# mikwieczorek/centroids-reid

Hardware: AMD Instinct MI355X
Metric: train_images_per_sec (higher is better)
Workload: dtype bf16; 1 GPU; ResNet50 256x128 CTL training step: fwd+bwd, centroid-triplet + center + xent, Adam + center SGD (BASELINE configs[1]); P=16, K=4, global_batch=64, num_classes=751, parallelism=single

## Files before the change

centroids-reid_amd/csrc/elementwise.hip:

```cpp
#include "conv_common.hpp"

#include "vec16.hpp"

template <int CW>
__global__ __launch_bounds__(1024) void bn2d_finalize_kernel(const float* __restrict__ partial, int rows, int C,
                                                            double count, float* __restrict__ rmean,
                                                            float* __restrict__ rvar, int training, float momentum,
                                                            float eps, const float* __restrict__ gamma,
                                                            const float* __restrict__ beta,
                                                            float* __restrict__ mean_out,
                                                            float* __restrict__ invstd_out,
                                                            float* __restrict__ scale_shift) {
  constexpr int RG = 1024 / CW;
  __shared__ double red[16][2][CW];
  const int cl = threadIdx.x % CW, rg = threadIdx.x / CW;
  const int c = blockIdx.x * CW + cl;
  if (!training) {
    if (rg == 0 && c < C) {
      const float mu = rmean[c], is = 1.0f / sqrtf(rvar[c] + eps);
      mean_out[c] = mu; invstd_out[c] = is;
      const float sc = is * (gamma ? gamma[c] : 1.f);
      scale_shift[c] = sc; scale_shift[C + c] = (beta ? beta[c] : 0.f) - mu * sc;
    }
    return;
// ... 472 lines not shown
    cb[k] = b.x; cb[k + 1] = b.y; cb[k + 2] = b.z; cb[k + 3] = b.w;
    cc[k] = c.x; cc[k + 1] = c.y; cc[k + 2] = c.z; cc[k + 3] = c.w;
  }
  if (!pg.dy && !act) {
    for (int64_t i = gtid; i < total; i += 2 * nthreads) {
      const int64_t i2 = i + nthreads;
      const bool two = i2 < total;
      float xv[V], gv[V], xw[V], gw[V];
      unsigned m1 = 0xffu, m2 = 0xffu;
      Vec16<T>::load(x + i * V, xv);
      Vec16<T>::load(g + i * V, gv);
      if (mask) m1 = mask[i];
      if (two) {
        Vec16<T>::load(x + i2 * V, xw);
        Vec16<T>::load(g + i2 * V, gw);
        if (mask) m2 = mask[i2];
      }
      float o[V];
#pragma unroll
      for (int k = 0; k < V; ++k) { gv[k] = ((m1 >> k) & 1u) ? gv[k] : 0.f; o[k] = fmaf(ca[k], gv[k], fmaf(cb[k], xv[k], cc[k])); }
      if (gm_out) Vec16<T>::store(gm_out + i * V, gv);
      Vec16<T>::store(dx + i * V, o);
      if (two) {
#pragma unroll
        for (int k = 0; k < V; ++k) { gw[k] = ((m2 >> k) & 1u) ? gw[k] : 0.f; o[k] = fmaf(ca[k], gw[k], fmaf(cb[k], xw[k], cc[k])); }
        if (gm_out) Vec16<T>::store(gm_out + i2 * V, gw);
        Vec16<T>::store(dx + i2 * V, o);
      }
    }
    return;
  }
  for (int64_t i = gtid; i < total; i += nthreads) {
    float xv[V], gv[V];
    Vec16<T>::load(x + i * V, xv);
    if (pg.dy) {
      const int64_t r = i / cpr;
      const int hw = pg.H * pg.W, bb = (int)(r / hw), rem = (int)(r - (int64_t)bb * hw);
      pool_grad_gather<T>(reinterpret_cast<const T*>(pg.dy), pg.idx, bb, rem / pg.W, rem % pg.W, (int)(i - r * cpr), pg.H / 2,
                          pg.W / 2, cpr, gv);
    } else {
      Vec16<T>::load(g + i * V, gv);
    }
    if (mask) {
      const unsigned m = mask[i];
#pragma unroll
      for (int k = 0; k < V; ++k) gv[k] = ((m >> k) & 1u) ? gv[k] : 0.f;
    } else if (act) {
      float av[V];
      Vec16<T>::load(act + i * V, av);
#pragma unroll
      for (int k = 0; k < V; ++k) gv[k] = av[k] > 0.f ? gv[k] : 0.f;
    }
    if (gm_out) Vec16<T>::store(gm_out + i * V, gv);
    float o[V];
#pragma unroll
    for (int k = 0; k < V; ++k) o[k] = fmaf(ca[k], gv[k], fmaf(cb[k], xv[k], cc[k]));
    Vec16<T>::store(dx + i * V, o);
  }
}

template <int V>
__device__ __forceinline__ void store_taps(uint8_t* p, const uint8_t (&bi)[V]) {
  static_assert(V == 4 || V == 8, "16-byte vectors of 4- or 2-byte elements");
  uint32_t lo = (uint32_t)bi[0] | ((uint32_t)bi[1] << 8) | ((uint32_t)bi[2] << 16) | ((uint32_t)bi[3] << 24);
  if constexpr (V == 4) {
    *reinterpret_cast<uint32_t*>(p) = lo;
  } else {
    uint32_t hi = (uint32_t)bi[4] | ((uint32_t)bi[5] << 8) | ((uint32_t)bi[6] << 16) | ((uint32_t)bi[7] << 24);
    *reinterpret_cast<uint2*>(p) = make_uint2(lo, hi);
  }
}
template <typename T>
__global__ __launch_bounds__(256) void maxpool_fwd_kernel(const T* __restrict__ x, int B, int H, int W, int C,
                                                          T* __restrict__ y, uint8_t* __restrict__ idx) {
  constexpr int V = Vec16<T>::N;
  const int OH = H / 2, OW = W / 2, cpr = C / V;
  const int64_t total = (int64_t)B * OH * OW * cpr;
  for (int64_t i = (int64_t)blockIdx.x * 256 + threadIdx.x; i < total; i += (int64_t)gridDim.x * 256) {
    int cc, ox, oy, b;
    if (total < (int64_t)1 << 31) {
      const unsigned u = (unsigned)i, q1 = u / (unsigned)cpr, q2 = q1 / (unsigned)OW;
      cc = (int)(u - q1 * cpr); ox = (int)(q1 - q2 * OW); b = (int)(q2 / (unsigned)OH); oy = (int)(q2 - (unsigned)b * OH);
    } else {
      cc = (int)(i % cpr);
      int64_t p = i / cpr;
      ox = (int)(p % OW); p /= OW;
      oy = (int)(p % OH);
      b = (int)(p / OH);
    }
    float best[V];
    uint8_t bi[V];
#pragma unroll
    for (int k = 0; k < V; ++k) { best[k] = -INFINITY; bi[k] = 0; }
#pragma unroll
    for (int r = 0; r < 3; ++r)
#pragma unroll
      for (int s = 0; s < 3; ++s) {
        const int iy = oy * 2 + r - 1, ix = ox * 2 + s - 1;
        if ((unsigned)iy < (unsigned)H && (unsigned)ix < (unsigned)W) {
          float v[V];
          Vec16<T>::load(x + (((int64_t)b * H + iy) * W + ix) * C + cc * V, v);
#pragma unroll
          for (int k = 0; k < V; ++k)
            if (v[k] > best[k]) { best[k] = v[k]; bi[k] = (uint8_t)(r * 3 + s); }
        }
      }
    Vec16<T>::store(y + i * V, best);
    if (idx) store_taps<V>(idx + i * V, bi);
  }
}

template <typename T>
__global__ __launch_bounds__(256) void bn_apply_maxpool_kernel(const T* __restrict__ x, const float* __restrict__ scale_shift,
                                                               int relu, int B, int H, int W, int C, T* __restrict__ y,
                                                               uint8_t* __restrict__ idx) {
  constexpr int V = Vec16<T>::N;
  const int OH = H / 2, OW = W / 2, cpr = C / V;
  const int64_t total = (int64_t)B * OH * OW * cpr;
  for (int64_t i = (int64_t)blockIdx.x * 256 + threadIdx.x; i < total; i += (int64_t)gridDim.x * 256) {
    int cc, ox, oy, b;
    if (total < (int64_t)1 << 31) {
      const unsigned u = (unsigned)i, q1 = u / (unsigned)cpr, q2 = q1 / (unsigned)OW;
      cc = (int)(u - q1 * cpr); ox = (int)(q1 - q2 * OW); b = (int)(q2 / (unsigned)OH); oy = (int)(q2 - (unsigned)b * OH);
    } else {
      cc = (int)(i % cpr);
      int64_t p = i / cpr;
      ox = (int)(p % OW); p /= OW;
      oy = (int)(p % OH);
      b = (int)(p / OH);
    }
    float sc[V], sh[V], best[V];
    uint8_t bi[V];
#pragma unroll
    for (int k = 0; k < V; ++k) { sc[k] = scale_shift[cc * V + k]; sh[k] = scale_shift[C + cc * V + k]; best[k] = -INFINITY; bi[k] = 0; }
#pragma unroll
    for (int r = 0; r < 3; ++r)
#pragma unroll
      for (int s = 0; s < 3; ++s) {
        const int iy = oy * 2 + r - 1, ix = ox * 2 + s - 1;
        if ((unsigned)iy < (unsigned)H && (unsigned)ix < (unsigned)W) {
          float v[V];
          Vec16<T>::load(x + (((int64_t)b * H + iy) * W + ix) * C + cc * V, v);
#pragma unroll
          for (int k = 0; k < V; ++k) {
            float yv = fmaf(v[k], sc[k], sh[k]);
            if (relu) yv = fmaxf(yv, 0.f);
            yv = Vec16<T>::rnd(yv);
            if (yv > best[k]) { best[k] = yv; bi[k] = (uint8_t)(r * 3 + s); }
          }
        }
      }
    Vec16<T>::store(y + i * V, best);
    if (idx) store_taps<V>(idx + i * V, bi);
  }
}

template <typename T>
__global__ __launch_bounds__(256) void maxpool_bwd_kernel(const T* __restrict__ dy, const uint8_t* __restrict__ idx,
                                                          int B, int H, int W, int C, T* __restrict__ dx) {
  constexpr int V = Vec16<T>::N;
  const int OH = H / 2, OW = W / 2, cpr = C / V;
  const int row = blockIdx.x;
  const int b = row / H, iy = row - b * H;
  T* drow = dx + (int64_t)row * W * C;
  const int nr = (iy & 1) ? 2 : 1;
  const int rr0 = (iy & 1) ? 0 : 1, rstep = 2;
  for (int par = 0; par < 2; ++par) {
    const int ns = par ? 2 : 1, ss0 = par ? 0 : 1;
    for (int v = threadIdx.x; v < (W / 2) * cpr; v += 256) {
      const int ix = 2 * (v / cpr) + par, cc = v % cpr;
      float acc[V];
#pragma unroll
      for (int k = 0; k < V; ++k) acc[k] = 0.f;
      for (int ri = 0; ri < nr; ++ri) {
        const int r = rr0 + ri * rstep, oy = (iy + 1 - r) >> 1;
        if (oy >= OH) continue;
        for (int si = 0; si < ns; ++si) {
          const int sx = ss0 + si * 2, ox = (ix + 1 - sx) >> 1;
          if (ox >= OW) continue;
          const int64_t o = ((((int64_t)b * OH + oy) * OW + ox) * cpr + cc) * V;
          float g[V];
          Vec16<T>::load(dy + o, g);
          uint8_t tap[V];
          if constexpr (V == 8) *reinterpret_cast<uint2*>(tap) = *reinterpret_cast<const uint2*>(idx + o);
          else *reinterpret_cast<unsigned*>(tap) = *reinterpret_cast<const unsigned*>(idx + o);
          const uint8_t want = (uint8_t)(r * 3 + sx);
#pragma unroll
          for (int k = 0; k < V; ++k) acc[k] += (tap[k] == want) ? g[k] : 0.f;
        }
      }
      Vec16<T>::store(drow + ((int64_t)ix * cpr + cc) * V, acc);
    }
  }
}

template <typename T>
__global__ __launch_bounds__(256) void gap_fwd_kernel(const T* __restrict__ x, int HW, int C, float* __restrict__ out,
                                                      int64_t* __restrict__ counter) {
  constexpr int V = Vec16<T>::N;
  __shared__ float red[8][32][V + 1];
  if (counter && blockIdx.x == 0 && blockIdx.y == 0 && threadIdx.x == 0) *counter += 1;
  const int cl = threadIdx.x & 31, rl = threadIdx.x >> 5;
  const int b = blockIdx.y, cc = blockIdx.x * 32 + cl;
  const bool live = cc * V < C;
  float acc[V];
#pragma unroll
  for (int k = 0; k < V; ++k) acc[k] = 0.f;
  if (live) {
    const T* p = x + (int64_t)b * HW * C + cc * V;
    for (int i = rl; i < HW; i += 8) {
      float v[V];
      Vec16<T>::load(p + (int64_t)i * C, v);
#pragma unroll
      for (int k = 0; k < V; ++k) acc[k] += v[k];
    }
  }
#pragma unroll
  for (int k = 0; k < V; ++k) red[rl][cl][k] = acc[k];
  __syncthreads();
  for (int e = threadIdx.x; e < 32 * V; e += 256) {
    const int c2 = e / V, k = e - c2 * V;
    const int ch = (blockIdx.x * 32 + c2) * V + k;
    if (ch < C) {
      float a = 0.f;
#pragma unroll
      for (int q = 0; q < 8; ++q) a += red[q][c2][k];
      out[(int64_t)b * C + ch] = a / (float)HW;
    }
  }
}

template <typename T>
__global__ __launch_bounds__(256) void gap_bwd_kernel(const float* __restrict__ dfeat, int HW, int C, int64_t total_chunks,
                                                      T* __restrict__ dx) {
  constexpr int V = Vec16<T>::N;
  const int cpr = C / V;
  const float inv = 1.0f / (float)HW;
  for (int64_t i = (int64_t)blockIdx.x * 256 + threadIdx.x; i < total_chunks; i += (int64_t)gridDim.x * 256) {
    int cc;
    int64_t b;
    if (total_chunks < (int64_t)1 << 31) { const unsigned u = (unsigned)i; cc = (int)(u % (unsigned)cpr); b = u / (unsigned)(cpr * HW); }
    else { cc = (int)(i % cpr); b = i / ((int64_t)cpr * HW); }
    float v[V];
#pragma unroll
    for (int k = 0; k < V; ++k) v[k] = dfeat[b * C + cc * V + k] * inv;
    Vec16<T>::store(dx + i * V, v);
  }
}

__device__ __forceinline__ void store_px4(float* p, const float (&v)[4]) { *reinterpret_cast<float4*>(p) = make_float4(v[0], v[1], v[2], v[3]); }
__device__ __forceinline__ void store_px4(unsigned short* p, const float (&v)[4]) {
  *reinterpret_cast<uint2*>(p) = make_uint2(Bf16T::pack2(v[0], v[1]), Bf16T::pack2(v[2], v[3]));
}
__device__ __forceinline__ void store_px4(_Float16* p, const float (&v)[4]) {
  *reinterpret_cast<uint2*>(p) = make_uint2(F16T::pack2(v[0], v[1]), F16T::pack2(v[2], v[3]));
}
template <typename T>
__global__ __launch_bounds__(256) void image_pad_kernel(const float* __restrict__ x, int B, int H, int W, T* __restrict__ y) {
  const int PH = H + 8, PW = W + 6;
  const int rows = B * PH;
  constexpr int RB = 8;
  if ((W & 3) == 0) {
    const int G = W / 4 + 2;
    for (int row0 = blockIdx.x * RB; row0 < rows; row0 += gridDim.x * RB) {
      const int n = min(RB, rows - row0) * G;
      for (int e = threadIdx.x; e < n; e += 256) {
        const int rl = e / G, gq = e - rl * G, row = row0 + rl;
        const int b = row / PH, py = row - b * PH, iy = py - 3;
        T* dst = y + (int64_t)row * PW * 4;
        const float z[4] = {0.f, 0.f, 0.f, 0.f};
        if (gq == 0 || gq == G - 1) {
          T* d = dst + (gq == 0 ? 0 : (W + 3) * 4);
          store_px4(d, z); store_px4(d + 4, z); store_px4(d + 8, z);
          continue;
        }
        const int ix = (gq - 1) * 4;
        float4 p0 = make_float4(0.f, 0.f, 0.f, 0.f), p1 = p0, p2 = p0;
        if ((unsigned)iy < (unsigned)H) {
          const float* src = x + (((int64_t)b * 3) * H + iy) * W + ix;
          p0 = *reinterpret_cast<const float4*>(src);
          p1 = *reinterpret_cast<const float4*>(src + (int64_t)H * W);
          p2 = *reinterpret_cast<const float4*>(src + (int64_t)2 * H * W);
        }
        T* d = dst + (ix + 3) * 4;
        const float v0[4] = {p0.x, p1.x, p2.x, 0.f}, v1[4] = {p0.y, p1.y, p2.y, 0.f};
        const float v2[4] = {p0.z, p1.z, p2.z, 0.f}, v3[4] = {p0.w, p1.w, p2.w, 0.f};
        store_px4(d, v0); store_px4(d + 4, v1); store_px4(d + 8, v2); store_px4(d + 12, v3);
      }
    }
    return;
  }
  for (int row0 = blockIdx.x * RB; row0 < rows; row0 += gridDim.x * RB) {
    const int n = min(RB, rows - row0) * PW;
    for (int e = threadIdx.x; e < n; e += 256) {
      const int rl = e / PW, px = e - rl * PW, row = row0 + rl;
      const int b = row / PH, py = row - b * PH, iy = py - 3, ix = px - 3;
      float v[4] = {0.f, 0.f, 0.f, 0.f};
      if ((unsigned)iy < (unsigned)H && (unsigned)ix < (unsigned)W) {
        const float* src = x + (((int64_t)b * 3) * H + iy) * W + ix;
#pragma unroll
        for (int c = 0; c < 3; ++c) v[c] = src[(int64_t)c * H * W];
      }
      store_px4(y + ((int64_t)row * PW + px) * 4, v);
    }
  }
}
// ... 76 lines not shown
      return;
    }
  }
  for (int tap = 0; tap < taps; ++tap) {
#pragma unroll
    for (int k = 0; k < 4; ++k) {
      const int o = o0 + ty + 8 * k, c = c0 + tx;
      tl[ty + 8 * k][tx] = (o < e.O && c < e.I) ? e.w[((int64_t)o * e.I + c) * taps + tap] : 0.f;
    }
    __syncthreads();
#pragma unroll
    for (int k = 0; k < 4; ++k) {
      const int o = o0 + ty + 8 * k, c = c0 + tx;
      if (o < e.O && c < e.I) ElemIO<T>::st(reinterpret_cast<T*>(e.krsc) + ((int64_t)o * taps + tap) * e.I + c, tl[ty + 8 * k][tx]);
      const int c2 = c0 + ty + 8 * k, o2 = o0 + tx;
      if (e.crsk && c2 < e.I && o2 < e.O)
        ElemIO<T>::st(reinterpret_cast<T*>(e.crsk) + ((int64_t)c2 * taps + tap) * e.O + o2, tl[tx][ty + 8 * k]);
    }
    __syncthreads();
  }
}

__device__ __forceinline__ void x3_split_bits(float v, unsigned short* hi, unsigned short* lo) {
  const unsigned short h = f32_to_bf16_bits(v);
  *hi = h;
  *lo = f32_to_bf16_bits(v - bf16_bits_to_f32(h));
}
__global__ __launch_bounds__(256) void weight_prep_x3_kernel(const float* __restrict__ w, int O, int I, int kh, int kw,
                                                             unsigned short* __restrict__ w2) {
  const int64_t total = (int64_t)O * I * kh * kw;
  for (int64_t i = (int64_t)blockIdx.x * 256 + threadIdx.x; i < total; i += (int64_t)gridDim.x * 256) {
    const int c = (int)(i % I);
    int64_t t = i / I;
    const int s = (int)(t % kw); t /= kw;
    const int r = (int)(t % kh);
    const int o = (int)(t / kh);
    x3_split_bits(w[(((int64_t)o * I + c) * kh + r) * kw + s], w2 + i, w2 + total + i);
  }
}
__global__ __launch_bounds__(256) void weight_prep_multi_x3_kernel(const WPrepEntry* __restrict__ tab, int n_ent,
                                                                   const int* __restrict__ tile_start) {
  int lo = 0, hi = n_ent - 1;
  const int bid = blockIdx.x;
  while (lo < hi) { const int mid = (lo + hi + 1) >> 1; if (tile_start[mid] <= bid) lo = mid; else hi = mid - 1; }
  const WPrepEntry e = tab[lo];
  const int tiles_c = (e.I + 31) / 32;
  const int tix = bid - tile_start[lo];
  const int o0 = (tix / tiles_c) * 32, c0 = (tix % tiles_c) * 32;
  const int tx = threadIdx.x & 31, ty = threadIdx.x >> 5;
  const int taps = e.kh * e.kw;
  const int64_t plane = (int64_t)e.O * taps * e.I;
  unsigned short* out = reinterpret_cast<unsigned short*>(e.krsc);
  for (int tap = 0; tap < taps; ++tap) {
#pragma unroll
    for (int k = 0; k < 4; ++k) {
      const int o = o0 + ty + 8 * k, c = c0 + tx;
      if (o < e.O && c < e.I) {
        const int64_t d = ((int64_t)o * taps + tap) * e.I + c;
        x3_split_bits(e.w[((int64_t)o * e.I + c) * taps + tap], out + d, out + plane + d);
      }
    }
  }
}
__global__ __launch_bounds__(256) void weight_prep_multi_x3_train_kernel(const WPrepEntry* __restrict__ tab, int n_ent,
                                                                         const int* __restrict__ tile_start) {
  __shared__ float tl[32][33];
  int lo = 0, hi = n_ent - 1;
  const int bid = blockIdx.x;
  while (lo < hi) { const int mid = (lo + hi + 1) >> 1; if (tile_start[mid] <= bid) lo = mid; else hi = mid - 1; }
  const WPrepEntry e = tab[lo];
  const int tiles_c = (e.I + 31) / 32;
  const int tix = bid - tile_start[lo];
  const int o0 = (tix / tiles_c) * 32, c0 = (tix % tiles_c) * 32;
  const int tx = threadIdx.x & 31, ty = threadIdx.x >> 5;
  const int taps = e.kh * e.kw;
  const int64_t plane = (int64_t)e.O * taps * e.I;
  unsigned short* krsc = reinterpret_cast<unsigned short*>(e.krsc);
  unsigned short* crsk = reinterpret_cast<unsigned short*>(e.crsk);
  for (int tap = 0; tap < taps; ++tap) {
#pragma unroll
    for (int k = 0; k < 4; ++k) {
      const int o = o0 + ty + 8 * k, c = c0 + tx;
      tl[ty + 8 * k][tx] = (o < e.O && c < e.I) ? e.w[((int64_t)o * e.I + c) * taps + tap] : 0.f;
    }
    __syncthreads();
#pragma unroll
    for (int k = 0; k < 4; ++k) {
      const int o = o0 + ty + 8 * k, c = c0 + tx;
      if (o < e.O && c < e.I) {
        const int64_t d = ((int64_t)o * taps + tap) * e.I + c;
        x3_split_bits(tl[ty + 8 * k][tx], krsc + d, krsc + plane + d);
      }
      const int c2 = c0 + ty + 8 * k, o2 = o0 + tx;
      if (c2 < e.I && o2 < e.O) {
        const int64_t d = ((int64_t)c2 * taps + tap) * e.O + o2;
        x3_split_bits(tl[tx][ty + 8 * k], crsk + d, crsk + plane + d);
      }
    }
    __syncthreads();
  }
}

template <typename T>
__global__ __launch_bounds__(256) void stem_weight_prep_kernel(const float* __restrict__ w, T* __restrict__ out) {
  const int i = blockIdx.x * 256 + threadIdx.x;
  if (i >= 64 * 256) return;
  const int o = i >> 8, k = i & 255, r = k >> 5, s = (k & 31) >> 2, c = k & 3;
  const float v = (r < 7 && s < 7 && c < 3) ? w[((o * 3 + c) * 7 + r) * 7 + s] : 0.f;
  ElemIO<T>::st(out + i, v);
}

template <typename T>
__global__ __launch_bounds__(256) void nhwc_to_nchw_kernel(const T* __restrict__ x, int B, int HW, int C, float* __restrict__ y) {
  const int64_t total = (int64_t)B * HW * C;
  for (int64_t i = (int64_t)blockIdx.x * 256 + threadIdx.x; i < total; i += (int64_t)gridDim.x * 256) {
    const int p = (int)(i % HW);
    const int c = (int)((i / HW) % C);
    const int64_t b = i / ((int64_t)HW * C);
    y[i] = ElemIO<T>::ld(x + (b * HW + p) * C + c);
  }
}

static inline unsigned ew_blocks_cap(int64_t total_threads_needed, int64_t mult, int64_t cap) {
  int64_t b = (total_threads_needed + 255) / 256;
  if (b > cap) b = cap;
  if (b < 1) b = 1;
  int64_t g = mult > 0 ? mult : 1, r = 256;
  while (r) { const int64_t t = g % r; g = r; r = t; }
  const int64_t q = mult > 0 ? mult / g : 1;
  b = (b + q - 1) / q * q;
  return (unsigned)b;
}
static inline int64_t ew_env_cap() {
  static const int64_t cap = [] { const char* e = getenv("CREID_EW_BLOCKS"); const int v = e ? atoi(e) : 0; return (int64_t)(v > 0 ? v : 0); }();
  return cap;
}
static inline unsigned ew_blocks(int64_t total_threads_needed, int64_t mult) {
  const int64_t e = ew_env_cap();
  return ew_blocks_cap(total_threads_needed, mult, e > 0 ? e : 2048);
}
template <auto KERNEL>
static inline unsigned ew_blocks_k(int64_t total_threads_needed, int64_t mult) {
  static const int64_t resident = [] {
    int per_cu = 0, dev = 0, ncu = 256;
    if (hipOccupancyMaxActiveBlocksPerMultiprocessor(&per_cu, KERNEL, 256, 0) != hipSuccess || per_cu <= 0) per_cu = 8;
    (void)hipGetDevice(&dev);
    if (hipDeviceGetAttribute(&ncu, hipDeviceAttributeMultiprocessorCount, dev) != hipSuccess || ncu <= 0) ncu = 256;
    return (int64_t)per_cu * ncu;
  }();
  const int64_t e = ew_env_cap();
  return ew_blocks_cap(total_threads_needed, mult, e > 0 ? e : resident);
}

#define DISPATCH_T(dtype, EXPR_F32, EXPR_BF16, EXPR_F16) \
  do {                                                  \
    if ((dtype) == CREID_F32) { EXPR_F32; }             \
    else if ((dtype) == CREID_BF16) { EXPR_BF16; }      \
    else if ((dtype) == CREID_F16) { EXPR_F16; }        \
    else return CREID_E_DTYPE;                          \
  } while (0)

static bool fin_dry(int bit) {
  static const int v = creid_ablation_env("CREID_BN_FIN_DRY");
  return (v & bit) != 0;
}
extern "C" {

int creid_bn2d_finalize(const float* partial, int64_t rows, int64_t C, int64_t count, float* running_mean,
                        float* running_var, int training, float momentum, float eps, const float* gamma,
                        const float* beta, float* mean_out, float* invstd_out, float* scale_shift, void* stream) {
  CREID_CHECK_ARG(C > 0 && mean_out && invstd_out && scale_shift &&
                  (training ? (partial && rows > 0 && count > 0) : (running_mean && running_var)));
  if (!fin_dry(1)) {
    if (C <= 256 && rows >= 512)
      hipLaunchKernelGGL(bn2d_finalize_kernel<4>, dim3((unsigned)((C + 3) / 4)), dim3(1024), 0, as_stream(stream), partial,
                         (int)rows, (int)C, (double)count, running_mean, running_var, training, momentum, eps, gamma, beta,
                         mean_out, invstd_out, scale_shift);
    else
      hipLaunchKernelGGL(bn2d_finalize_kernel<16>, dim3((unsigned)((C + 15) / 16)), dim3(1024), 0, as_stream(stream), partial,
                         (int)rows, (int)C, (double)count, running_mean, running_var, training, momentum, eps, gamma, beta,
                         mean_out, invstd_out, scale_shift);
  }
  CREID_LAUNCH_RET();
}

int64_t creid_col_stats_rows(int64_t M) { int64_t r = (M + 127) / 128; return r < 1 ? 1 : r; }

int creid_col_stats(const void* x, int64_t M, int64_t C, int dtype, float* partial, void* stream) {
  CREID_CHECK_ARG(x && partial && M > 0 && C > 0 && C % 8 == 0);
  const int rows = (int)creid_col_stats_rows(M);
  hipStream_t s = as_stream(stream);
  DISPATCH_T(dtype,
             hipLaunchKernelGGL(col_stats_kernel<float>, dim3((unsigned)((C / 4 + 31) / 32), rows), dim3(256), 0, s,
                                (const float*)x, M, (int)C, 128, partial),
             hipLaunchKernelGGL(col_stats_kernel<unsigned short>, dim3((unsigned)((C / 8 + 31) / 32), rows), dim3(256), 0,
                                s, (const unsigned short*)x, M, (int)C, 128, partial),
             hipLaunchKernelGGL(col_stats_kernel<_Float16>, dim3((unsigned)((C / 8 + 31) / 32), rows), dim3(256), 0,
                                s, (const _Float16*)x, M, (int)C, 128, partial));
  CREID_LAUNCH_RET();
}

int creid_bn2d_apply_mask(const void* x, const float* scale_shift, const void* residual, int relu, int64_t M, int64_t C,
                          int dtype, void* y, uint8_t* mask_out, void* stream) {
  CREID_CHECK_ARG(x && scale_shift && y && M > 0 && C > 0 && C % 8 == 0);
  if (mask_out && dtype == CREID_F32) return CREID_E_DTYPE;
  hipStream_t s = as_stream(stream);
  DISPATCH_T(dtype,
             hipLaunchKernelGGL(bn2d_apply_kernel<float>, dim3(ew_blocks_k<bn2d_apply_kernel<float>>(M * C / 4, C / 4)), dim3(256), 0, s,
                                (const float*)x, scale_shift, (const float*)residual, relu, M, (int)C, (float*)y,
                                (uint8_t*)nullptr, (const float*)nullptr),
             hipLaunchKernelGGL(bn2d_apply_kernel<unsigned short>, dim3(ew_blocks_k<bn2d_apply_kernel<unsigned short>>(M * C / 8, C / 8)), dim3(256), 0, s,
                                (const unsigned short*)x, scale_shift, (const unsigned short*)residual, relu, M,
                                (int)C, (unsigned short*)y, mask_out, (const float*)nullptr),
             hipLaunchKernelGGL(bn2d_apply_kernel<_Float16>, dim3(ew_blocks_k<bn2d_apply_kernel<_Float16>>(M * C / 8, C / 8)), dim3(256), 0, s,
                                (const _Float16*)x, scale_shift, (const _Float16*)residual, relu, M,
                                (int)C, (_Float16*)y, mask_out, (const float*)nullptr));
  CREID_LAUNCH_RET();
}

int creid_bn2d_finalize_apply_mask(const float* partial, int64_t rows, int64_t C, int64_t M, float* running_mean,
                                   float* running_var, float momentum, float eps, const float* gamma, const float* beta,
                                   float* mean_out, float* invstd_out, float* scale_shift, const void* x, const void* residual,
                                   int relu, int dtype, void* y, uint8_t* mask_out, int row_blocks, void* stream) {
  CREID_CHECK_ARG(partial && rows > 0 && C > 0 && M > 0 && mean_out && invstd_out && scale_shift && x && y);
  if (mask_out && dtype == CREID_F32) return CREID_E_DTYPE;
  const int64_t strip = dtype == CREID_F32 ? 32 : 64;
  if (C % strip != 0 || rows > 1024) return CREID_E_SHAPE;
  const int strips = (int)(C / strip);
  int rb = row_blocks > 0 ? row_blocks : (512 + strips - 1) / strips;
  if (row_blocks <= 0) { if (rb > 32) rb = 32; if (rb < 4) rb = 4; }
  int64_t rpb = ((M + rb - 1) / rb + 31) / 32 * 32;
  rb = (int)((M + rpb - 1) / rpb);
  hipStream_t s = as_stream(stream);
  const dim3 grid((unsigned)strips, (unsigned)rb);
  DISPATCH_T(dtype,
             hipLaunchKernelGGL(bn2d_fin_apply_kernel<float>, grid, dim3(256), 0, s, (const float*)x, partial, (int)rows, (int)C, M,
                                (double)M, running_mean, running_var, momentum, eps, gamma, beta, mean_out, invstd_out, scale_shift,
                                (const float*)residual, relu, (float*)y, (uint8_t*)nullptr, (int)rpb),
             hipLaunchKernelGGL(bn2d_fin_apply_kernel<unsigned short>, grid, dim3(256), 0, s, (const unsigned short*)x, partial,
                                (int)rows, (int)C, M, (double)M, running_mean, running_var, momentum, eps, gamma, beta, mean_out,
                                invstd_out, scale_shift, (const unsigned short*)residual, relu, (unsigned short*)y, mask_out,
                                (int)rpb),
             hipLaunchKernelGGL(bn2d_fin_apply_kernel<_Float16>, grid, dim3(256), 0, s, (const _Float16*)x, partial, (int)rows,
                                (int)C, M, (double)M, running_mean, running_var, momentum, eps, gamma, beta, mean_out, invstd_out,
                                scale_shift, (const _Float16*)residual, relu, (_Float16*)y, mask_out, (int)rpb));
  CREID_LAUNCH_RET();
}

int creid_bn2d_apply_dual_mask(const void* x, const float* scale_shift, const void* x_res, const float* scale_shift_res, int relu,
                               int64_t M, int64_t C, int dtype, void* y, uint8_t* mask_out, void* stream) {
  CREID_CHECK_ARG(x && scale_shift && x_res && scale_shift_res && y && M > 0 && C > 0 && C % 8 == 0);
  if (mask_out && dtype == CREID_F32) return CREID_E_DTYPE;
  hipStream_t s = as_stream(stream);
  DISPATCH_T(dtype,
             hipLaunchKernelGGL(bn2d_apply_kernel<float>, dim3(ew_blocks_k<bn2d_apply_kernel<float>>(M * C / 4, C / 4)), dim3(256), 0, s,
                                (const float*)x, scale_shift, (const float*)x_res, relu, M, (int)C, (float*)y,
                                (uint8_t*)nullptr, scale_shift_res),
             hipLaunchKernelGGL(bn2d_apply_kernel<unsigned short>, dim3(ew_blocks_k<bn2d_apply_kernel<unsigned short>>(M * C / 8, C / 8)), dim3(256), 0, s,
                                (const unsigned short*)x, scale_shift, (const unsigned short*)x_res, relu, M,
                                (int)C, (unsigned short*)y, mask_out, scale_shift_res),
             hipLaunchKernelGGL(bn2d_apply_kernel<_Float16>, dim3(ew_blocks_k<bn2d_apply_kernel<_Float16>>(M * C / 8, C / 8)), dim3(256), 0, s,
                                (const _Float16*)x, scale_shift, (const _Float16*)x_res, relu, M,
                                (int)C, (_Float16*)y, mask_out, scale_shift_res));
  CREID_LAUNCH_RET();
}

int creid_bn2d_apply(const void* x, const float* scale_shift, const void* residual, int relu, int64_t M, int64_t C,
                     int dtype, void* y, void* stream) {
  return creid_bn2d_apply_mask(x, scale_shift, residual, relu, M, C, dtype, y, nullptr, stream);
}

int64_t creid_bn2d_bwd_rows(int64_t M) { int64_t r = (M + 127) / 128; return r < 1 ? 1 : r; }

struct Reduce2 { const void* x2; const float* mean2; const float* invstd2; float* partial2; };

static int bn2d_bwd_impl(const void* x, const void* g, const void* act, const uint8_t* mask, PoolGrad pg, const float* mean,
                         const float* invstd, const float* gamma, int64_t M, int64_t C, int dtype, float* partial,
                         int partial_ready, float* sums, float* dgamma_accum, float* dbeta_accum, void* dx, void* gm_out,
                         void* stream, Reduce2 r2 = Reduce2{nullptr, nullptr, nullptr, nullptr}) {
  CREID_CHECK_ARG(x && (g || pg.dy) && mean && invstd && (partial || partial_ready == 2) && sums && dx && M > 0 && C > 0 && C % 8 == 0);
  if (mask && dtype == CREID_F32) return CREID_E_DTYPE;
  const int rows = (int)creid_bn2d_bwd_rows(M);
  hipStream_t s = as_stream(stream);
  if (!partial_ready)
  DISPATCH_T(dtype,
             hipLaunchKernelGGL(bn2d_bwd_reduce_kernel<float>, dim3((unsigned)((C / 4 + 31) / 32), rows), dim3(256), 0, s,
                                (const float*)x, (const float*)g, (const float*)act, mean, invstd, M, (int)C, 128, partial,
                                (const uint8_t*)nullptr, pg),
             hipLaunchKernelGGL(bn2d_bwd_reduce_kernel<unsigned short>, dim3((unsigned)((C / 8 + 31) / 32), rows), dim3(256),
                                0, s, (const unsigned short*)x, (const unsigned short*)g, (const unsigned short*)act, mean,
                                invstd, M, (int)C, 128, partial, mask, pg),
             hipLaunchKernelGGL(bn2d_bwd_reduce_kernel<_Float16>, dim3((unsigned)((C / 8 + 31) / 32), rows), dim3(256),
                                0, s, (const _Float16*)x, (const _Float16*)g, (const _Float16*)act, mean,
                                invstd, M, (int)C, 128, partial, mask, pg));
  if (partial_ready != 2 && !fin_dry(2)) {
    if (C <= 256 && rows >= 512)
      hipLaunchKernelGGL(bn2d_bwd_finalize_kernel<4>, dim3((unsigned)((C + 3) / 4)), dim3(1024), 0, s, partial, rows, (int)C,
                         (double)M, mean, invstd, gamma, sums, dgamma_accum, dbeta_accum);
    else
      hipLaunchKernelGGL(bn2d_bwd_finalize_kernel<16>, dim3((unsigned)((C + 15) / 16)), dim3(1024), 0, s, partial, rows, (int)C,
                         (double)M, mean, invstd, gamma, sums, dgamma_accum, dbeta_accum);
  }
  if (r2.x2) {
    if (act || gm_out || pg.dy || dtype == CREID_F32) return CREID_E_ARG;
    const dim3 grid2((unsigned)((C / 8 + 31) / 32), (unsigned)rows);
    if (dtype == CREID_BF16)
      hipLaunchKernelGGL(bn2d_bwd_apply_reduce2_kernel<unsigned short>, grid2, dim3(256), 0, s, (const unsigned short*)x,
                         (const unsigned short*)g, mask, sums, M, (int)C, 128, (unsigned short*)dx, (const unsigned short*)r2.x2,
                         r2.mean2, r2.invstd2, r2.partial2);
    else
      hipLaunchKernelGGL(bn2d_bwd_apply_reduce2_kernel<_Float16>, grid2, dim3(256), 0, s, (const _Float16*)x, (const _Float16*)g,
                         mask, sums, M, (int)C, 128, (_Float16*)dx, (const _Float16*)r2.x2, r2.mean2, r2.invstd2, r2.partial2);
    CREID_LAUNCH_RET();
  }
  DISPATCH_T(dtype,
             hipLaunchKernelGGL(bn2d_bwd_apply_kernel<float>, dim3(ew_blocks_k<bn2d_bwd_apply_kernel<float>>(M * C / 4, C / 4)), dim3(256), 0, s,
                                (const float*)x, (const float*)g, (const float*)act, sums, M, (int)C,
                                (float*)dx, (float*)gm_out, (const uint8_t*)nullptr, pg),
             hipLaunchKernelGGL(bn2d_bwd_apply_kernel<unsigned short>, dim3(ew_blocks_k<bn2d_bwd_apply_kernel<unsigned short>>(M * C / 8, C / 8)), dim3(256), 0, s,
                                (const unsigned short*)x, (const unsigned short*)g, (const unsigned short*)act, sums, M,
                                (int)C, (unsigned short*)dx, (unsigned short*)gm_out, mask, pg),
             hipLaunchKernelGGL(bn2d_bwd_apply_kernel<_Float16>, dim3(ew_blocks_k<bn2d_bwd_apply_kernel<_Float16>>(M * C / 8, C / 8)), dim3(256), 0, s,
                                (const _Float16*)x, (const _Float16*)g, (const _Float16*)act, sums, M,
                                (int)C, (_Float16*)dx, (_Float16*)gm_out, mask, pg));
  CREID_LAUNCH_RET();
}

int creid_bn2d_bwd_mask(const void* x, const void* g, const void* act, const uint8_t* mask, const float* mean,
                        const float* invstd, const float* gamma, int64_t M, int64_t C, int dtype, float* partial,
                        int partial_ready, float* sums, float* dgamma_accum, float* dbeta_accum, void* dx, void* gm_out,
                        void* stream) {
  CREID_CHECK_ARG(g);
  return bn2d_bwd_impl(x, g, act, mask, PoolGrad{nullptr, nullptr, 0, 0}, mean, invstd, gamma, M, C, dtype, partial, partial_ready,
                       sums, dgamma_accum, dbeta_accum, dx, gm_out, stream);
}

int creid_bn2d_bwd_mask_reduce2(const void* x, const void* g, const uint8_t* mask, const float* mean, const float* invstd,
                                const float* gamma, int64_t M, int64_t C, int dtype, float* partial, int partial_ready, float* sums,
                                float* dgamma_accum, float* dbeta_accum, void* dx, const void* x2, const float* mean2,
                                const float* invstd2, float* partial2, void* stream) {
  CREID_CHECK_ARG(g && x2 && mean2 && invstd2 && partial2);
  if (!creid_is16(dtype)) return CREID_E_DTYPE;
  return bn2d_bwd_impl(x, g, nullptr, mask, PoolGrad{nullptr, nullptr, 0, 0}, mean, invstd, gamma, M, C, dtype, partial, partial_ready,
                       sums, dgamma_accum, dbeta_accum, dx, nullptr, stream, Reduce2{x2, mean2, invstd2, partial2});
}

int creid_bn2d_bwd_pooled(const void* x, const void* dy_pooled, const uint8_t* idx, int64_t B, int64_t H, int64_t W,
                          const void* act, const float* mean, const float* invstd, const float* gamma, int64_t C, int dtype,
                          float* partial, float* sums, float* dgamma_accum, float* dbeta_accum, void* dx, void* stream) {
  CREID_CHECK_ARG(dy_pooled && idx && B > 0 && H > 0 && W > 0 && H % 2 == 0 && W % 2 == 0);
  return bn2d_bwd_impl(x, nullptr, act, nullptr, PoolGrad{dy_pooled, idx, (int)H, (int)W}, mean, invstd, gamma, B * H * W, C, dtype,
                       partial, 0, sums, dgamma_accum, dbeta_accum, dx, nullptr, stream);
}

int creid_bn2d_apply_maxpool3x3s2(const void* x, const float* scale_shift, int relu, int64_t B, int64_t H, int64_t W, int64_t C,
                                  int dtype, void* y, uint8_t* idx, void* stream) {
  CREID_CHECK_ARG(x && scale_shift && y && idx && B > 0 && H > 0 && W > 0 && C % 8 == 0 && H % 2 == 0 && W % 2 == 0);
  hipStream_t s = as_stream(stream);
  DISPATCH_T(dtype,
             hipLaunchKernelGGL(bn_apply_maxpool_kernel<float>, dim3(ew_blocks(B * H * W * C / 16, 1)), dim3(256), 0, s,
                                (const float*)x, scale_shift, relu, (int)B, (int)H, (int)W, (int)C, (float*)y, idx),
             hipLaunchKernelGGL(bn_apply_maxpool_kernel<unsigned short>, dim3(ew_blocks(B * H * W * C / 32, 1)), dim3(256), 0, s,
                                (const unsigned short*)x, scale_shift, relu, (int)B, (int)H, (int)W, (int)C, (unsigned short*)y,
                                idx),
             hipLaunchKernelGGL(bn_apply_maxpool_kernel<_Float16>, dim3(ew_blocks(B * H * W * C / 32, 1)), dim3(256), 0, s,
                                (const _Float16*)x, scale_shift, relu, (int)B, (int)H, (int)W, (int)C, (_Float16*)y,
                                idx));
  CREID_LAUNCH_RET();
}

int creid_bn2d_bwd(const void* x, const void* g, const void* act, const float* mean, const float* invstd,
                   const float* gamma, int64_t M, int64_t C, int dtype, float* partial, int partial_ready, float* sums,
                   float* dgamma_accum, float* dbeta_accum, void* dx, void* gm_out, void* stream) {
  return creid_bn2d_bwd_mask(x, g, act, nullptr, mean, invstd, gamma, M, C, dtype, partial, partial_ready, sums, dgamma_accum,
                             dbeta_accum, dx, gm_out, stream);
}

int creid_maxpool3x3s2_fwd(const void* x, int64_t B, int64_t H, int64_t W, int64_t C, int dtype, void* y, uint8_t* idx,
                           void* stream) {
  CREID_CHECK_ARG(x && y && B > 0 && H > 0 && W > 0 && C % 8 == 0 && H % 2 == 0 && W % 2 == 0);
  hipStream_t s = as_stream(stream);
  DISPATCH_T(dtype,
             hipLaunchKernelGGL(maxpool_fwd_kernel<float>, dim3(ew_blocks(B * H * W * C / 16, 1)), dim3(256), 0, s,
                                (const float*)x, (int)B, (int)H, (int)W, (int)C, (float*)y, idx),
             hipLaunchKernelGGL(maxpool_fwd_kernel<unsigned short>, dim3(ew_blocks(B * H * W * C / 32, 1)), dim3(256), 0, s,
                                (const unsigned short*)x, (int)B, (int)H, (int)W, (int)C, (unsigned short*)y, idx),
             hipLaunchKernelGGL(maxpool_fwd_kernel<_Float16>, dim3(ew_blocks(B * H * W * C / 32, 1)), dim3(256), 0, s,
                                (const _Float16*)x, (int)B, (int)H, (int)W, (int)C, (_Float16*)y, idx));
  CREID_LAUNCH_RET();
}

int creid_maxpool3x3s2_bwd(const void* dy, const uint8_t* idx, int64_t B, int64_t H, int64_t W, int64_t C, int dtype,
                           void* dx, void* stream) {
  CREID_CHECK_ARG(dy && dx && idx && B > 0 && H > 0 && W > 0 && C % 8 == 0 && H % 2 == 0 && W % 2 == 0);
  hipStream_t s = as_stream(stream);
  DISPATCH_T(dtype,
             hipLaunchKernelGGL(maxpool_bwd_kernel<float>, dim3((unsigned)(B * H)), dim3(256), 0, s,
                                (const float*)dy, idx, (int)B, (int)H, (int)W, (int)C, (float*)dx),
             hipLaunchKernelGGL(maxpool_bwd_kernel<unsigned short>, dim3((unsigned)(B * H)), dim3(256), 0, s,
                                (const unsigned short*)dy, idx, (int)B, (int)H, (int)W, (int)C, (unsigned short*)dx),
             hipLaunchKernelGGL(maxpool_bwd_kernel<_Float16>, dim3((unsigned)(B * H)), dim3(256), 0, s,
                                (const _Float16*)dy, idx, (int)B, (int)H, (int)W, (int)C, (_Float16*)dx));
  CREID_LAUNCH_RET();
}

static int gap_fwd_impl(const void* x, int64_t B, int64_t HW, int64_t C, int dtype, float* feat, int64_t* counter, void* stream) {
  CREID_CHECK_ARG(x && feat && B > 0 && HW > 0 && C % 8 == 0);
  hipStream_t s = as_stream(stream);
  DISPATCH_T(dtype,
             hipLaunchKernelGGL(gap_fwd_kernel<float>, dim3((unsigned)((C / 4 + 31) / 32), (unsigned)B), dim3(256), 0, s,
                                (const float*)x, (int)HW, (int)C, feat, counter),
             hipLaunchKernelGGL(gap_fwd_kernel<unsigned short>, dim3((unsigned)((C / 8 + 31) / 32), (unsigned)B),
                                dim3(256), 0, s, (const unsigned short*)x, (int)HW, (int)C, feat, counter),
             hipLaunchKernelGGL(gap_fwd_kernel<_Float16>, dim3((unsigned)((C / 8 + 31) / 32), (unsigned)B),
                                dim3(256), 0, s, (const _Float16*)x, (int)HW, (int)C, feat, counter));
  CREID_LAUNCH_RET();
}

int creid_gap_fwd(const void* x, int64_t B, int64_t HW, int64_t C, int dtype, float* feat, void* stream) {
  return gap_fwd_impl(x, B, HW, C, dtype, feat, nullptr, stream);
}

int creid_gap_fwd_count(const void* x, int64_t B, int64_t HW, int64_t C, int dtype, float* feat, int64_t* forward_counter,
                        void* stream) {
  CREID_CHECK_ARG(forward_counter);
  return gap_fwd_impl(x, B, HW, C, dtype, feat, forward_counter, stream);
}

int creid_gap_bwd(const float* dfeat, int64_t B, int64_t HW, int64_t C, int dtype, void* dx, void* stream) {
  CREID_CHECK_ARG(dfeat && dx && B > 0 && HW > 0 && C % 8 == 0);
  hipStream_t s = as_stream(stream);
  DISPATCH_T(dtype,
             hipLaunchKernelGGL(gap_bwd_kernel<float>, dim3(ew_blocks(B * HW * C / 4, 1)), dim3(256), 0, s, dfeat, (int)HW,
                                (int)C, B * HW * C / 4, (float*)dx),
             hipLaunchKernelGGL(gap_bwd_kernel<unsigned short>, dim3(ew_blocks(B * HW * C / 8, 1)), dim3(256), 0, s, dfeat,
                                (int)HW, (int)C, B * HW * C / 8, (unsigned short*)dx),
             hipLaunchKernelGGL(gap_bwd_kernel<_Float16>, dim3(ew_blocks(B * HW * C / 8, 1)), dim3(256), 0, s, dfeat,
                                (int)HW, (int)C, B * HW * C / 8, (_Float16*)dx));
  CREID_LAUNCH_RET();
}

int creid_image_to_nhwc4_pad(const float* x_nchw, int64_t B, int64_t H, int64_t W, int dtype, void* xpad, void* stream) {
  CREID_CHECK_ARG(x_nchw && xpad && B > 0 && H > 0 && W > 0);
  hipStream_t s = as_stream(stream);
  const int64_t total = B * (H + 8) * (W + 6);
  DISPATCH_T(dtype,
             hipLaunchKernelGGL(image_pad_kernel<float>, dim3(ew_blocks(total, 1)), dim3(256), 0, s, x_nchw, (int)B, (int)H,
                                (int)W, (float*)xpad),
             hipLaunchKernelGGL(image_pad_kernel<unsigned short>, dim3(ew_blocks(total, 1)), dim3(256), 0, s, x_nchw, (int)B,
                                (int)H, (int)W, (unsigned short*)xpad),
             hipLaunchKernelGGL(image_pad_kernel<_Float16>, dim3(ew_blocks(total, 1)), dim3(256), 0, s, x_nchw, (int)B,
                                (int)H, (int)W, (_Float16*)xpad));
  CREID_LAUNCH_RET();
}

int creid_weight_prep(const float* w_oihw, int64_t O, int64_t I, int64_t kh, int64_t kw, int dtype, void* w_krsc,
                      void* w_crsk, void* stream) {
  CREID_CHECK_ARG(w_oihw && w_krsc && O > 0 && I > 0 && kh > 0 && kw > 0);
  hipStream_t s = as_stream(stream);
  const int64_t total = O * I * kh * kw;
  if (dtype == CREID_BF16X3) {
    CREID_CHECK_ARG(!w_crsk);
    hipLaunchKernelGGL(weight_prep_x3_kernel, dim3(ew_blocks(total, 1)), dim3(256), 0, s, w_oihw, (int)O, (int)I, (int)kh,
                       (int)kw, (unsigned short*)w_krsc);
    CREID_LAUNCH_RET();
  }
  DISPATCH_T(dtype,
             hipLaunchKernelGGL(weight_prep_kernel<float>, dim3(ew_blocks(total, 1)), dim3(256), 0, s, w_oihw, (int)O, (int)I,
                                (int)kh, (int)kw, (float*)w_krsc, (float*)w_crsk),
             hipLaunchKernelGGL(weight_prep_kernel<unsigned short>, dim3(ew_blocks(total, 1)), dim3(256), 0, s, w_oihw,
                                (int)O, (int)I, (int)kh, (int)kw, (unsigned short*)w_krsc, (unsigned short*)w_crsk),
             hipLaunchKernelGGL(weight_prep_kernel<_Float16>, dim3(ew_blocks(total, 1)), dim3(256), 0, s, w_oihw,
                                (int)O, (int)I, (int)kh, (int)kw, (_Float16*)w_krsc, (_Float16*)w_crsk));
  CREID_LAUNCH_RET();
}

int64_t creid_weight_prep_entry_bytes(void) { return (int64_t)sizeof(WPrepEntry); }

int creid_weight_prep_multi(const void* table_dev, const int32_t* tile_start_dev, int64_t n_entries, int64_t total_tiles,
                            int dtype, void* stream) {
  CREID_CHECK_ARG(table_dev && tile_start_dev && n_entries > 0 && total_tiles > 0);
  hipStream_t s = as_stream(stream);
  if (dtype == CREID_BF16X3) {
    hipLaunchKernelGGL(weight_prep_multi_x3_kernel, dim3((unsigned)total_tiles), dim3(256), 0, s, (const WPrepEntry*)table_dev,
                       (int)n_entries, tile_start_dev);
    CREID_LAUNCH_RET();
  }
  DISPATCH_T(dtype,
             hipLaunchKernelGGL(weight_prep_multi_kernel<float>, dim3((unsigned)total_tiles), dim3(256), 0, s,
                                (const WPrepEntry*)table_dev, (int)n_entries, tile_start_dev),
             hipLaunchKernelGGL(weight_prep_multi_kernel<unsigned short>, dim3((unsigned)total_tiles), dim3(256), 0, s,
                                (const WPrepEntry*)table_dev, (int)n_entries, tile_start_dev),
             hipLaunchKernelGGL(weight_prep_multi_kernel<_Float16>, dim3((unsigned)total_tiles), dim3(256), 0, s,
                                (const WPrepEntry*)table_dev, (int)n_entries, tile_start_dev));
  CREID_LAUNCH_RET();
}

int creid_weight_prep_x3_train_multi(const void* table_dev, const int32_t* tile_start_dev, int64_t n_entries,
                                     int64_t total_tiles, void* stream) {
  CREID_CHECK_ARG(table_dev && tile_start_dev && n_entries > 0 && total_tiles > 0);
  hipLaunchKernelGGL(weight_prep_multi_x3_train_kernel, dim3((unsigned)total_tiles), dim3(256), 0, as_stream(stream),
                     (const WPrepEntry*)table_dev, (int)n_entries, tile_start_dev);
  CREID_LAUNCH_RET();
}

int64_t creid_bn2d_fold_entry_bytes(void) { return (int64_t)sizeof(BnFoldEntry); }

int creid_bn2d_fold_multi(const void* table_dev, int64_t n_entries, void* stream) {
  CREID_CHECK_ARG(table_dev && n_entries > 0 && n_entries < (1 << 20));
  hipLaunchKernelGGL(bn_fold_multi_kernel, dim3((unsigned)n_entries, 8), dim3(256), 0, as_stream(stream),
                     (const BnFoldEntry*)table_dev);
  CREID_LAUNCH_RET();
}

int creid_stem_weight_prep(const float* w_oihw, int dtype, void* w_stem, void* stream) {
  CREID_CHECK_ARG(w_oihw && w_stem);
  hipStream_t s = as_stream(stream);
  DISPATCH_T(dtype,
             hipLaunchKernelGGL(stem_weight_prep_kernel<float>, dim3(64), dim3(256), 0, s, w_oihw, (float*)w_stem),
             hipLaunchKernelGGL(stem_weight_prep_kernel<unsigned short>, dim3(64), dim3(256), 0, s, w_oihw,
                                (unsigned short*)w_stem),
             hipLaunchKernelGGL(stem_weight_prep_kernel<_Float16>, dim3(64), dim3(256), 0, s, w_oihw,
                                (_Float16*)w_stem));
  CREID_LAUNCH_RET();
}

int creid_nhwc_to_nchw_f32(const void* x, int64_t B, int64_t HW, int64_t C, int dtype, float* y, void* stream) {
  CREID_CHECK_ARG(x && y && B > 0 && HW > 0 && C > 0);
  hipStream_t s = as_stream(stream);
  DISPATCH_T(dtype,
             hipLaunchKernelGGL(nhwc_to_nchw_kernel<float>, dim3(ew_blocks(B * HW * C, 1)), dim3(256), 0, s, (const float*)x,
                                (int)B, (int)HW, (int)C, y),
             hipLaunchKernelGGL(nhwc_to_nchw_kernel<unsigned short>, dim3(ew_blocks(B * HW * C, 1)), dim3(256), 0, s,
                                (const unsigned short*)x, (int)B, (int)HW, (int)C, y),
             hipLaunchKernelGGL(nhwc_to_nchw_kernel<_Float16>, dim3(ew_blocks(B * HW * C, 1)), dim3(256), 0, s,
                                (const _Float16*)x, (int)B, (int)HW, (int)C, y));
  CREID_LAUNCH_RET();
}

}

template <typename T>
__global__ __launch_bounds__(256) void ibn_col_stats_kernel(const T* __restrict__ x, int HW, int C, int rows_per_block,
                                                            int rpi, float* __restrict__ partial) {
  constexpr int V = Vec16<T>::N;
  __shared__ float red[2][256 * V];
  const int cpr = C / V, cw = cpr < 32 ? cpr : 32, nrl = 256 / cw;
  const int cch = threadIdx.x % cw, rl = threadIdx.x / cw;
// ... 422 lines not shown
```

Baseline: 11210 images/s.

## Add strip-based fused BN+maxpool forward and quad-gather maxpool backward kernels

Adds a forward kernel where each thread walks a vertical strip of output rows, reusing the overlapping input row between neighbouring 3x3/stride-2 windows instead of reloading all nine taps per output. Also adds a backward kernel where each thread owns a 2x2 input quad and gathers contributions from up to four outputs, replacing the row-parallel scatter kernel. Both are enabled by default behind environment knobs, with a heuristic choosing strip length from the available parallelism. Longer strips give fewer threads and more serial dependency per thread, which could hurt occupancy on the stem-layer shapes.

```diff
diff --git a/centroids-reid_amd/csrc/elementwise.hip b/centroids-reid_amd/csrc/elementwise.hip
--- a/centroids-reid_amd/csrc/elementwise.hip
+++ b/centroids-reid_amd/csrc/elementwise.hip
@@ -648,6 +648,172 @@
       }
     Vec16<T>::store(y + i * V, best);
     if (idx) store_taps<V>(idx + i * V, bi);
+  }
+}
+
+template <typename T> __device__ __forceinline__ void vec16_unpack(const uint4& t, float (&v)[Vec16<T>::N]);
+template <> __device__ __forceinline__ void vec16_unpack<float>(const uint4& t, float (&v)[4]) {
+  v[0] = __uint_as_float(t.x); v[1] = __uint_as_float(t.y); v[2] = __uint_as_float(t.z); v[3] = __uint_as_float(t.w);
+}
+template <> __device__ __forceinline__ void vec16_unpack<unsigned short>(const uint4& t, float (&v)[8]) {
+  const unsigned w[4] = {t.x, t.y, t.z, t.w};
+#pragma unroll
+  for (int i = 0; i < 4; ++i) { v[2 * i] = __uint_as_float(w[i] << 16); v[2 * i + 1] = __uint_as_float(w[i] & 0xffff0000u); }
+}
+template <> __device__ __forceinline__ void vec16_unpack<_Float16>(const uint4& t, float (&v)[8]) {
+  const unsigned w[4] = {t.x, t.y, t.z, t.w};
+#pragma unroll
+  for (int i = 0; i < 4; ++i) { v[2 * i] = F16T::lo(w[i]); v[2 * i + 1] = F16T::hi(w[i]); }
+}
+
+template <typename T>
+__device__ __forceinline__ void pool_row_max(const uint4 (&raw)[3], const float (&sc)[Vec16<T>::N], const float (&sh)[Vec16<T>::N],
+                                             int relu, bool left_ok, bool row_ok, float (&m)[Vec16<T>::N], int (&si)[Vec16<T>::N]) {
+  constexpr int V = Vec16<T>::N;
+#pragma unroll
+  for (int k = 0; k < V; ++k) { m[k] = -INFINITY; si[k] = 0; }
+#pragma unroll
+  for (int s = 0; s < 3; ++s) {
+    float v[V];
+    vec16_unpack<T>(raw[s], v);
+    const bool ok = row_ok && (s > 0 || left_ok);
+#pragma unroll
+    for (int k = 0; k < V; ++k) {
+      float yv = fmaf(v[k], sc[k], sh[k]);
+      if (relu) yv = fmaxf(yv, 0.f);
+      yv = Vec16<T>::rnd(yv);
+      const float cv = ok ? yv : -INFINITY;
+      const bool win = cv > m[k];
+      m[k] = win ? cv : m[k];
+      si[k] = win ? s : si[k];
+    }
+  }
+}
+
+template <typename T>
+__global__ __launch_bounds__(256) void bn_apply_maxpool_strip_kernel(const T* __restrict__ x, const float* __restrict__ scale_shift,
+                                                                     int relu, int B, int H, int W, int C, T* __restrict__ y,
+                                                                     uint8_t* __restrict__ idx, int R) {
+  constexpr int V = Vec16<T>::N;
+  const int OH = H / 2, OW = W / 2, cpr = C / V, strips = (OH + R - 1) / R;
+  const int64_t total = (int64_t)B * strips * OW * cpr;
+  for (int64_t i = (int64_t)blockIdx.x * 256 + threadIdx.x; i < total; i += (int64_t)gridDim.x * 256) {
+    int cc, ox, st, b;
+    if (total < (int64_t)1 << 31) {
+      const unsigned u = (unsigned)i, q1 = u / (unsigned)cpr, q2 = q1 / (unsigned)OW;
+      cc = (int)(u - q1 * cpr); ox = (int)(q1 - q2 * OW); b = (int)(q2 / (unsigned)strips); st = (int)(q2 - (unsigned)b * strips);
+    } else {
+      cc = (int)(i % cpr);
+      int64_t p = i / cpr;
+      ox = (int)(p % OW); p /= OW;
+      st = (int)(p % strips);
+      b = (int)(p / strips);
+    }
+    const int oy0 = st * R, n = min(R, OH - oy0);
+    float sc[V], sh[V];
+#pragma unroll
+    for (int k = 0; k < V; ++k) { sc[k] = scale_shift[cc * V + k]; sh[k] = scale_shift[C + cc * V + k]; }
+    const bool left_ok = ox > 0;
+    const int64_t c_left = (int64_t)max(2 * ox - 1, 0) * C, c_mid = (int64_t)(2 * ox) * C;
+    const T* xb = x + (int64_t)b * H * W * C + cc * V;
+    auto load_row = [&](int iy, uint4 (&raw)[3]) {
+      const T* p = xb + (int64_t)iy * W * C;
+      raw[0] = *reinterpret_cast<const uint4*>(p + c_left);
+      raw[1] = *reinterpret_cast<const uint4*>(p + c_mid);
+      raw[2] = *reinterpret_cast<const uint4*>(p + c_mid + C);
+    };
+    uint4 rt[3], ra[3], rb[3];
+    load_row(max(2 * oy0 - 1, 0), rt);
+    load_row(2 * oy0, ra);
+    load_row(2 * oy0 + 1, rb);
+    float m0[V];
+    int s0[V];
+    pool_row_max<T>(rt, sc, sh, relu, left_ok, oy0 > 0, m0, s0);
+    for (int j = 0; j < n; ++j) {
+      uint4 na[3], nb[3];
+      const int oyn = min(oy0 + j + 1, OH - 1);
+      load_row(2 * oyn, na);
+      load_row(2 * oyn + 1, nb);
+      float best[V], mr[V];
+      int t[V], sr[V];
+      uint8_t bi[V];
+#pragma unroll
+      for (int k = 0; k < V; ++k) {
+        best[k] = -INFINITY; t[k] = 0;
+        const bool w0 = m0[k] > best[k];
+        best[k] = w0 ? m0[k] : best[k]; t[k] = w0 ? s0[k] : t[k];
+      }
+      pool_row_max<T>(ra, sc, sh, relu, left_ok, true, mr, sr);
+#pragma unroll
+      for (int k = 0; k < V; ++k) {
+        const bool w1 = mr[k] > best[k];
+        best[k] = w1 ? mr[k] : best[k]; t[k] = w1 ? 3 + sr[k] : t[k];
+      }
+      pool_row_max<T>(rb, sc, sh, relu, left_ok, true, m0, s0);
+#pragma unroll
+      for (int k = 0; k < V; ++k) {
+        const bool w2 = m0[k] > best[k];
+        best[k] = w2 ? m0[k] : best[k]; t[k] = w2 ? 6 + s0[k] : t[k];
+        bi[k] = (uint8_t)t[k];
+      }
+      const int64_t o = ((((int64_t)b * OH + oy0 + j) * OW + ox) * cpr + cc) * V;
+      Vec16<T>::store(y + o, best);
+      if (idx) store_taps<V>(idx + o, bi);
+#pragma unroll
+      for (int s = 0; s < 3; ++s) { ra[s] = na[s]; rb[s] = nb[s]; }
+    }
+  }
+}
+
+template <typename T>
+__global__ __launch_bounds__(256) void maxpool_bwd_quad_kernel(const T* __restrict__ dy, const uint8_t* __restrict__ idx,
+                                                               int B, int H, int W, int C, T* __restrict__ dx) {
+  constexpr int V = Vec16<T>::N;
+  const int OH = H / 2, OW = W / 2, cpr = C / V;
+  const int64_t total = (int64_t)B * OH * OW * cpr;
+  for (int64_t i = (int64_t)blockIdx.x * 256 + threadIdx.x; i < total; i += (int64_t)gridDim.x * 256) {
+    int cc, ox, oy, b;
+    if (total < (int64_t)1 << 31) {
+      const unsigned u = (unsigned)i, q1 = u / (unsigned)cpr, q2 = q1 / (unsigned)OW;
+      cc = (int)(u - q1 * cpr); ox = (int)(q1 - q2 * OW); b = (int)(q2 / (unsigned)OH); oy = (int)(q2 - (unsigned)b * OH);
+    } else {
+      cc = (int)(i % cpr);
+      int64_t p = i / cpr;
+      ox = (int)(p % OW); p /= OW;
+      oy = (int)(p % OH);
+      b = (int)(p / OH);
+    }
+    const bool right = ox + 1 < OW, below = oy + 1 < OH;
+    const int ox1 = right ? ox + 1 : ox, oy1 = below ? oy + 1 : oy;
+    const int64_t wy[2] = {((int64_t)b * OH + oy) * OW, ((int64_t)b * OH + oy1) * OW};
+    const int wx[2] = {ox, ox1};
+    float g[2][2][V];
+    alignas(8) uint8_t tap[2][2][V];
+#pragma unroll
+    for (int a = 0; a < 2; ++a)
+#pragma unroll
+      for (int c = 0; c < 2; ++c) {
+        const int64_t o = ((wy[a] + wx[c]) * cpr + cc) * V;
+        Vec16<T>::load(dy + o, g[a][c]);
+        if constexpr (V == 8) *reinterpret_cast<uint2*>(tap[a][c]) = *reinterpret_cast<const uint2*>(idx + o);
+        else *reinterpret_cast<unsigned*>(tap[a][c]) = *reinterpret_cast<const unsigned*>(idx + o);
+      }
+    auto take = [&](int a, int c, bool live, int want, int k) {
+      return (live && tap[a][c][k] == (uint8_t)want) ? g[a][c][k] : 0.f;
+    };
+    float p00[V], p01[V], p10[V], p11[V];
+#pragma unroll
+    for (int k = 0; k < V; ++k) {
+      p00[k] = 0.f + take(0, 0, true, 4, k);
+      p01[k] = (0.f + take(0, 1, right, 3, k)) + take(0, 0, true, 5, k);
+      p10[k] = (0.f + take(1, 0, below, 1, k)) + take(0, 0, true, 7, k);
+      p11[k] = (((0.f + take(1, 1, below && right, 0, k)) + take(1, 0, below, 2, k)) + take(0, 1, right, 6, k)) + take(0, 0, true, 8, k);
+    }
+    T* d = dx + ((((int64_t)b * H + 2 * oy) * W + 2 * ox) * cpr + cc) * V;
+    Vec16<T>::store(d, p00);
+    Vec16<T>::store(d + C, p01);
+    Vec16<T>::store(d + (int64_t)W * C, p10);
+    Vec16<T>::store(d + (int64_t)W * C + C, p11);
   }
 }
 
@@ -1030,6 +1196,18 @@
   return ew_blocks_cap(total_threads_needed, mult, e > 0 ? e : resident);
 }
 
+static int pool_strip_rows(int64_t B, int64_t OH, int64_t per_row) {
+  const char* e = CREID_KNOB_ENV("CREID_POOL_STRIP");
+  if (e) return atoi(e) < 0 ? 0 : atoi(e);
+  for (int rows = 8; rows > 2; rows /= 2)
+    if (B * ((OH + rows - 1) / rows) * per_row >= 2 * 256 * 256) return rows;
+  return 2;
+}
+static bool pool_bwd_quad() {
+  const char* e = CREID_KNOB_ENV("CREID_POOL_BWD_QUAD");
+  return !e || atoi(e) != 0;
+}
+
 #define DISPATCH_T(dtype, EXPR_F32, EXPR_BF16, EXPR_F16) \
   do {                                                  \
     if ((dtype) == CREID_F32) { EXPR_F32; }             \
@@ -1235,6 +1413,18 @@
                                   int dtype, void* y, uint8_t* idx, void* stream) {
   CREID_CHECK_ARG(x && scale_shift && y && idx && B > 0 && H > 0 && W > 0 && C % 8 == 0 && H % 2 == 0 && W % 2 == 0);
   hipStream_t s = as_stream(stream);
+  const int64_t OH = H / 2, per_row = W / 2 * (C / (dtype == CREID_F32 ? 4 : 8));
+  if (const int rows = pool_strip_rows(B, OH, per_row)) {
+    const unsigned grid = ew_blocks(B * ((OH + rows - 1) / rows) * per_row, 1);
+    DISPATCH_T(dtype,
+               hipLaunchKernelGGL(bn_apply_maxpool_strip_kernel<float>, dim3(grid), dim3(256), 0, s, (const float*)x, scale_shift, relu,
+                                  (int)B, (int)H, (int)W, (int)C, (float*)y, idx, rows),
+               hipLaunchKernelGGL(bn_apply_maxpool_strip_kernel<unsigned short>, dim3(grid), dim3(256), 0, s, (const unsigned short*)x,
+                                  scale_shift, relu, (int)B, (int)H, (int)W, (int)C, (unsigned short*)y, idx, rows),
+               hipLaunchKernelGGL(bn_apply_maxpool_strip_kernel<_Float16>, dim3(grid), dim3(256), 0, s, (const _Float16*)x, scale_shift,
+                                  relu, (int)B, (int)H, (int)W, (int)C, (_Float16*)y, idx, rows));
+    CREID_LAUNCH_RET();
+  }
   DISPATCH_T(dtype,
              hipLaunchKernelGGL(bn_apply_maxpool_kernel<float>, dim3(ew_blocks(B * H * W * C / 16, 1)), dim3(256), 0, s,
                                 (const float*)x, scale_shift, relu, (int)B, (int)H, (int)W, (int)C, (float*)y, idx),
@@ -1272,6 +1462,16 @@
                            void* dx, void* stream) {
   CREID_CHECK_ARG(dy && dx && idx && B > 0 && H > 0 && W > 0 && C % 8 == 0 && H % 2 == 0 && W % 2 == 0);
   hipStream_t s = as_stream(stream);
+  if (pool_bwd_quad()) {
+    DISPATCH_T(dtype,
+               hipLaunchKernelGGL(maxpool_bwd_quad_kernel<float>, dim3(ew_blocks(B * H * W * C / 16, 1)), dim3(256), 0, s,
+                                  (const float*)dy, idx, (int)B, (int)H, (int)W, (int)C, (float*)dx),
+               hipLaunchKernelGGL(maxpool_bwd_quad_kernel<unsigned short>, dim3(ew_blocks(B * H * W * C / 32, 1)), dim3(256), 0, s,
+                                  (const unsigned short*)dy, idx, (int)B, (int)H, (int)W, (int)C, (unsigned short*)dx),
+               hipLaunchKernelGGL(maxpool_bwd_quad_kernel<_Float16>, dim3(ew_blocks(B * H * W * C / 32, 1)), dim3(256), 0, s,
+                                  (const _Float16*)dy, idx, (int)B, (int)H, (int)W, (int)C, (_Float16*)dx));
+    CREID_LAUNCH_RET();
+  }
   DISPATCH_T(dtype,
              hipLaunchKernelGGL(maxpool_bwd_kernel<float>, dim3((unsigned)(B * H)), dim3(256), 0, s,
                                 (const float*)dy, idx, (int)B, (int)H, (int)W, (int)C, (float*)dx),
```

After: 11220 images/s (median of 4 runs). No clear change (+0.1%).
